# acerbilab/pyvbmc

Measured on AMD Instinct MI355X. Metric: ELBO+entropy evals/sec at D=10, K=50, N=400, Ns=1e6 (1e6-sample-equivalent evals/s), higher is better.
Workload: dtype f64; 1 GPU; BASELINE config 3 per GPU: D=10 K=50 N=400 S=1, Ns=1000000 MC samples per GPU (job Ns=1000000), value+grad _neg_elcbo with soft bounds, eps=philox; parallelism=single GPU

## Files before the change

### pyvbmc_amd/_lib.py

```python
import ctypes as C
import os
import sys
import threading
from pathlib import Path

import numpy as np

_HERE = Path(__file__).resolve().parent
LIB_PATH = Path(os.environ.get("VBMC_HIP_LIB", _HERE / "libvbmc_hip.so"))

EPS_RESIDENT, EPS_PHILOX = 0, 1
MEAN_ZERO, MEAN_CONST, MEAN_NEGQUAD = 0, 1, 2
E_ARG, E_HIP, E_RCCL, E_NODEV, E_UNSUP, E_NONFINITE = -1, -2, -3, -4, -5, -6
E_NOTPD = -8
W_GP_CHANGED = 1
W_NOT_FUSED = 2
T_ENTMC, T_GLJ, T_PDF, T_PREDICT, T_ELBO, T_PREDICT_VAR, T_GP_POST, T_IS_MCMC = range(8)


class VbmcHipError(RuntimeError):
    def __init__(self, code, msg):
        super().__init__(f"libvbmc_hip error {code}: {msg}")
        self.code = code

# ... 272 lines not shown
            if rc == E_ARG:
                raise ValueError(msg)
            if rc == E_NODEV:
                raise NoDeviceError(rc, msg)
            if rc == E_NOTPD:
                raise np.linalg.LinAlgError(msg)
            raise VbmcHipError(rc, msg)

    def device_info(self):
        name = C.create_string_buffer(256)
        cu, clk, mem = C.c_int(), C.c_int(), C.c_uint64()
        self.check(self._lib.vbmc_device_info(self._h, name, 256, C.byref(cu), C.byref(clk), C.byref(mem)))
        return {"name": name.value.decode(), "cu_count": cu.value, "clock_khz": clk.value,
                "hbm_bytes": mem.value}

    def host_affinity(self):
        b, n = C.c_int(), C.c_int()
        self.check(self._lib.vbmc_host_affinity(self._h, C.byref(b), C.byref(n)))
        return bool(b.value), n.value

    def synchronize(self):
        self.check(self._lib.vbmc_synchronize(self._h))

    def set_timing(self, on):
        self.check(self._lib.vbmc_set_timing(self._h, int(on) if on else 0))

    def set_option(self, key, value):
        self.check(self._lib.vbmc_set_option(self._h, key.encode(), int(value)))

    def last_entmc_plan(self):
        out = (C.c_int * 4)()
        self.check(self._lib.vbmc_last_entmc_plan(self._h, out))
        return {"kernel": ("valu", "ws", "small", "mfma", "adam_fused", "ws", "ws")[out[0]] if out[0] >= 0 else None, "rg": out[1],
                "chunks": out[2], "resident_draws": bool(out[3]), "span": out[0] in (5, 6), "adam_tail": out[0] == 6}

    def philox_normals(self, K, n_half, D, seed, row_begin=0, row_count=None):
        row_count = n_half - row_begin if row_count is None else row_count
        out = np.empty((K, row_count, D))
        self.check(self._lib.vbmc_philox_normals(self._h, K, n_half, D, C.c_uint64(seed), row_begin, row_count, ptr(out)))
        return out

    def armed_stats(self):
        out = (C.c_uint64 * 6)()
        self.check(self._lib.vbmc_armed_stats(self._h, out))
        return dict(zip(("hits", "cancels", "late", "ident_checked", "ident_bad", "lost"), (int(v) for v in out)))

    def last_elbo_raw(self, D, K):
        out = np.empty(1 + D * K + 2 * K + D)
        self.check(self._lib.vbmc_last_elbo_raw(self._h, ptr(out), out.size))
        return out

    def last_kernel_ms(self, which=T_ENTMC):
        v = C.c_double()
        self.check(self._lib.vbmc_last_kernel_ms(self._h, which, C.byref(v)))
        return v.value

    def last_host_us(self):
        out = np.zeros(5)
        self.check(self._lib.vbmc_last_host_us(self._h, ptr(out)))
        return out

    def last_step_marks(self):
        out = np.zeros(4)
        self.check(self._lib.vbmc_last_step_marks(self._h, ptr(out)))
        return {"gp_word_us": out[0], "entropy_word_us": out[1],
                "gp_sums_in": ("prep launch", "finish launch", "entropy launch")[int(out[2])]}

# ... 108 lines not shown
```

### pyvbmc_amd/csrc/common.h

```cpp
#pragma once
#include <hip/hip_runtime.h>
#include <chrono>

#include <cstdint>
#include <cstdio>
#include <string>
#include <vector>

#include "../../include/vbmc_hip.h"
#include "scratch.h"

struct ncclComm;

struct MixLayout {
  int D = 0, K = 0;
  int o_mup = 0;
  int o_mu = 0;
  int o_is2 = 0;
  int o_wc = 0;
  int o_rc = 0;
  int o_lrc = 0;
  int o_sig = 0;
  int o_w = 0;
  int o_lam = 0;
// ... 179 lines not shown
  size_t h_eps_cap = 0;
  size_t h_pinned_cap = 0;
  double* h_pack = nullptr;
  size_t h_pack_cap = 0;
  bool pack_in_flight = false;
  bool pack_valid = false;
  bool defer_mix_upload = false;
  double* hp_dev = nullptr;
  int timing = 0;
  double host_us[5] = {0, 0, 0, 0, 0};
  double step_marks[4] = {0, 0, 0, 0};
  int gp_where = 0;
  int opt_entmc_valu = 0;
  int opt_gp_ship = 1;
  int opt_entmc_mfma = 1;
  int opt_elbo_pregen = 1;
  int opt_elbo_ahead = 1;
  int opt_predict_dma = 1;
  int opt_predict_fused = 1;
  int opt_arm_late_test = 0;
  int opt_acq_poll = 1;
  int opt_is_mcmc_threads = 512;
  void (*release_cb)(void*) = nullptr;
  void* release_cb_user = nullptr;
  int opt_adam_fused = 1;
  int opt_adam_tail = 1;
  int opt_ident_test = 0;
  bool ident_retry = false;
  int opt_elbo_arm = 1;
  bool counted = false;
  int opt_ws_span = 1;
  int opt_ws_front = 0;
  int opt_ws_pad = -1;
  int opt_mix_bar = 1;
  double* h_pack_dev = nullptr;
  double* h_pack_dev_of = nullptr;
  std::vector<double> exp_eta;
  double exp_eta_sum = 0.0;
  bool exp_eta_valid = false;
  int last_plan[4] = {-1, 0, 0, 0};
  size_t last_raw_off = 0;
  int last_raw_n = 0;

  GpState gp;
  GpState gp_next;
  double* d_post_ws = nullptr;
  size_t d_post_ws_cap = 0;

  ncclComm* comm = nullptr;
  int rank = 0, world = 1;

  std::vector<const double*> gp_watch_ptrs;
  std::vector<int64_t> gp_watch_lens;
  uint64_t gp_watch_ck = 0;

  ElboScratch elbo;
  void* adam = nullptr;
  void* acq_is = nullptr;
  bool host_bound = false;
  int host_cpus = 0;
  void* randn_dev = nullptr;
  int randn_last_reused = 0;
  int opt_randn_dev = 1;
  void* xf = nullptr;
};
inline int ctx_cus(const vbmc_ctx* ctx) { return ctx->prop.multiProcessorCount > 0 ? ctx->prop.multiProcessorCount : 256; }
// ... 292 lines not shown
```

### pyvbmc_amd/csrc/ctx.hip

```cpp
#include <algorithm>
#include <cmath>
#include <cstdarg>
#include <cstdlib>
#include <cstring>

#include <sched.h>

#include <cctype>
#include <cstdio>

#include "common.h"

thread_local std::string g_create_err;

int vbmc_fail(vbmc_ctx* ctx, int code, const char* fmt, ...) {
  char buf[1024];
  va_list ap;
  va_start(ap, fmt);
  vsnprintf(buf, sizeof buf, fmt, ap);
  va_end(ap);
  if (ctx)
    ctx->err = buf;
  else
    g_create_err = buf;
// ... 57 lines not shown
  HIP_TRY(ctx, stream_wait(ctx));
  for (int i = 0; dst && i < k; ++i)
    if (dst[i]) memcpy(dst[i] + o, ctx->h_pinned + i * stride, sizeof(double) * count);
  return 0;
}

#include <atomic>
static std::atomic<int> g_live_ctx[64];
int vbmc_live_contexts_on(int device) { return device >= 0 && device < 64 ? g_live_ctx[device].load() : 2; }

static void options_from_env(vbmc_ctx* c) {
  const char* e = getenv("VBMC_ENTMC_KERNEL");
  c->opt_entmc_valu = (e && e[0] == 'v') ? 1 : 0;
  e = getenv("VBMC_ELBO_PREGEN");
  c->opt_elbo_pregen = !(e && e[0] == '0');
  e = getenv("VBMC_ELBO_AHEAD");
  c->opt_elbo_ahead = !(e && e[0] == '0');
  e = getenv("VBMC_ELBO_ARM");
  c->opt_elbo_arm = e ? atoi(e) : 1;
  e = getenv("VBMC_ACQ_POLL");
  c->opt_acq_poll = !(e && e[0] == '0');
  e = getenv("VBMC_ADAM_FUSED");
  c->opt_adam_fused = e ? atoi(e) : 1;
  e = getenv("VBMC_RANDN_DEVICE");
  c->opt_randn_dev = e ? (e[0] == '0' ? 0 : e[0] == '2' ? 2 : 1) : 1;
  e = getenv("VBMC_ADAM_TAIL");
  c->opt_adam_tail = e ? atoi(e) : 1;
  e = getenv("VBMC_WS_SPAN");
  c->opt_ws_span = !(e && e[0] == '0');
  e = getenv("VBMC_WS_FRONT");
  if (e) c->opt_ws_front = atoi(e);
  e = getenv("VBMC_WS_PAD");
  if (e) c->opt_ws_pad = atoi(e);
  e = getenv("VBMC_MIX_BAR");
  c->opt_mix_bar = !(e && e[0] == '0');
  e = getenv("VBMC_PREDICT_DMA");
  c->opt_predict_dma = !(e && e[0] == '0');
  e = getenv("VBMC_PREDICT_FUSED_FINISH");
  if (e) c->opt_predict_fused = atoi(e);
  e = getenv("VBMC_GP_SHIP");
  c->opt_gp_ship = !(e && e[0] == '0');
}

extern "C" {

int vbmc_abi_version(void) { return 2; }

int vbmc_device_count(int* n_out) {
  int n = 0;
  hipError_t e = hipGetDeviceCount(&n);
  if (e != hipSuccess) {
    n = 0;
    (void)hipGetLastError();
  }
  if (n_out) *n_out = n;
  return VBMC_OK;
}

}

static void bind_host_thread(vbmc_ctx* ctx) {
  const char* e = getenv("VBMC_HOST_AFFINITY");
  if (e && e[0] == '0') return;
  char bus[64] = {0};
  if (hipDeviceGetPCIBusId(bus, (int)sizeof(bus) - 1, ctx->device) != hipSuccess) {
    (void)hipGetLastError();
// ... 152 lines not shown
  if (clock_khz) *clock_khz = ctx->prop.clockRate;
  if (hbm_bytes) *hbm_bytes = (uint64_t)ctx->prop.totalGlobalMem;
  return VBMC_OK;
}

int vbmc_synchronize(vbmc_ctx* ctx) {
  if (!ctx) return VBMC_E_ARG;
  if (ctx->device < 0) return VBMC_OK;
  HIP_TRY(ctx, hipSetDevice(ctx->device));
  HIP_TRY(ctx, stream_wait(ctx));
  return VBMC_OK;
}

int vbmc_set_option(vbmc_ctx* ctx, const char* key, int value) {
  if (!ctx || !key) return VBMC_E_ARG;
  if (!strcmp(key, "arm_late_test")) {
    ctx->opt_arm_late_test = value;
    return VBMC_OK;
  }
  if (!strcmp(key, "ident_test")) {
    ctx->opt_ident_test = value;
    return VBMC_OK;
  }
  spec_disarm(ctx);
  if (!strcmp(key, "entmc_kernel")) ctx->opt_entmc_valu = value == 1;
  else if (!strcmp(key, "entmc_mfma")) ctx->opt_entmc_mfma = value != 0;
  else if (!strcmp(key, "gp_ship")) ctx->opt_gp_ship = value != 0;
  else if (!strcmp(key, "elbo_pregen")) ctx->opt_elbo_pregen = value != 0;
  else if (!strcmp(key, "elbo_ahead")) ctx->opt_elbo_ahead = value != 0;
  else if (!strcmp(key, "predict_dma")) ctx->opt_predict_dma = value != 0;
  else if (!strcmp(key, "predict_fused")) ctx->opt_predict_fused = value < 0 ? 0 : value > 2 ? 2 : value;
  else if (!strcmp(key, "mix_bar")) ctx->opt_mix_bar = value != 0;
  else if (!strcmp(key, "ws_span")) ctx->opt_ws_span = value != 0;
  else if (!strcmp(key, "ws_pad")) ctx->opt_ws_pad = value > 8 ? 8 : value;
  else if (!strcmp(key, "ws_front")) ctx->opt_ws_front = value < 0 ? 0 : value > 990 ? 990 : value;
  else if (!strcmp(key, "elbo_arm")) ctx->opt_elbo_arm = value < 0 ? 0 : value > 2 ? 2 : value;
  else if (!strcmp(key, "acq_poll")) ctx->opt_acq_poll = value != 0;
  else if (!strcmp(key, "is_mcmc_threads")) ctx->opt_is_mcmc_threads = value <= 256 ? 256 : value >= 768 ? 768 : 512;
  else if (!strcmp(key, "randn_device")) ctx->opt_randn_dev = value < 0 ? 0 : value > 3 ? 3 : value;
  else if (!strcmp(key, "adam_tail")) ctx->opt_adam_tail = value;
  else if (!strcmp(key, "adam_fused")) ctx->opt_adam_fused = value;
  else return vbmc_fail(ctx, VBMC_E_ARG, "vbmc_set_option: unknown key '%s'", key);
  return VBMC_OK;
}

int vbmc_set_gp_watch(vbmc_ctx* ctx, const double* const* ptrs, const int64_t* lens, int n, uint64_t expected) {
  if (!ctx || n < 0 || (n > 0 && (!ptrs || !lens))) return VBMC_E_ARG;
  ctx->gp_watch_ptrs.assign(ptrs, ptrs + n);
  ctx->gp_watch_lens.assign(lens, lens + n);
  ctx->gp_watch_ck = expected;
  return VBMC_OK;
}

int vbmc_host_checksum(const double* const* ptrs, const int64_t* lens, int n, uint64_t* out) {
  if (!ptrs || !lens || n < 0 || !out) return VBMC_E_ARG;
  uint64_t s = 0;
  for (int a = 0; a < n; ++a) {
    if (!ptrs[a] || lens[a] < 0) return VBMC_E_ARG;
    s += (pack_checksum(ptrs[a], (size_t)lens[a]) + (uint64_t)lens[a]) * (0xD1B54A32D192ED03ull + 2ull * (uint64_t)a);
  }
  *out = s;
  return VBMC_OK;
}

int vbmc_last_entmc_plan(const vbmc_ctx* ctx, int out[4]) {
  if (!ctx || !out) return VBMC_E_ARG;
// ... 413 lines not shown
```

### pyvbmc_amd/csrc/entropy.hip

```cpp
#include <cstdlib>

#include <algorithm>

#include "common.h"
#include "fastmath.h"
#include "entropy_args.h"
#include "philox.h"
#ifdef FIN_TIMES
__device__ unsigned long long g_glj_stamp;
#define GLJ_STAMP() (g_glj_stamp = wall_clock64())
#endif
#include "glj_block.h"

namespace {

constexpr int WG = 256;
constexpr int WAVES = WG / 64;

__device__ inline double wave_sum(double v) {
  return fm::wave_sum_dpp(v);
}


template <int DP>
// ... 350 lines not shown
  a.row_count = row_count;
  a.seed = seed;
  a.eps_mode = eps_mode;
  a.want_grad = want_grad;
  const bool ws = use_ws_kernel(ctx, D, K);
  const int cus = ctx_cus(ctx);
  p.inv_ns = 1.0 / (double)ns_per_comp;
  int rows_per_wg = WG;
  a.rg = 1;
  size_t n_table = 0;
  if (ws) {
    const int64_t total_rows = row_count * K;
    int64_t rg = (total_rows + 64 * 2 * cus - 1) / (64 * 2 * cus);
    if (rg < 1) rg = 1;
    if (rg > 16) rg = 16;
    a.rg = (int)rg;
    rows_per_wg = 64 * a.rg;
    n_table = (size_t)K * (size_t)ws_table_rows(K) * (size_t)(p.DP + 6);
  }
  a.chunks = (int)((row_count + rows_per_wg - 1) / rows_per_wg);
  if (a.chunks < 1) a.chunks = 1;
  if (ws) {
    const int64_t slots = (int64_t)cus * ws_min_waves(p.DP, ws_ktmax_for(K), want_grad != 0);
    const int64_t fit = slots / K;
    if (fit >= 1 && a.chunks > fit && (int64_t)K * (a.chunks - 1) <= slots) {
      const int64_t rg2 = (row_count + 64 * fit - 1) / (64 * fit);
      if (rg2 <= 24) {
        a.rg = (int)rg2;
        rows_per_wg = 64 * a.rg;
        a.chunks = (int)((row_count + rows_per_wg - 1) / rows_per_wg);
      }
    }
  }
  a.pair_cus = 0;
  if (ws) {
    const int64_t total = (int64_t)K * a.chunks;
    if (ws_min_waves(p.DP, ws_ktmax_for(K), want_grad != 0) == 2 && total > cus && total <= 2 * (int64_t)cus)
      a.pair_cus = cus;
  }
  EntArgs at_launch = a;
  {
    const size_t n_eps = (size_t)K * (size_t)row_count * D;
    if (eps_mode == VBMC_EPS_PHILOX && ctx->opt_elbo_pregen && n_eps > 0 && n_eps <= ((size_t)1 << 28)) {
      at_launch.eps_mode = VBMC_EPS_RESIDENT;
      at_launch.eps = (const double*)ctx;
    }
    if (at_launch.eps_mode == VBMC_EPS_RESIDENT && at_launch.eps == nullptr) at_launch.eps = (const double*)ctx;
  }
  p.kernel = !ws                                                          ? EntKernel::Valu
             : entmc_small_applies(at_launch, p.DP)                       ? EntKernel::Small
             : ctx->opt_entmc_mfma && entmc_mfma_applies(at_launch, p.DP) ? EntKernel::Mfma
                                                                          : EntKernel::Ws;
  a.sp = WsSpan();
  a.gp_wgs = 0;
  p.gp_in_ws = false;
  if (p.kernel == EntKernel::Ws && ctx->opt_ws_span) {
    const int waves = ws_min_waves(p.DP, ws_ktmax_for(K), want_grad != 0);
    WsSpan sp;
    sp.cus = cus;
    sp.nb = (int)((row_count + 63) >> 6);
    sp.pad = ctx->opt_ws_pad >= 0 ? ctx->opt_ws_pad : 3;
    sp.T = (int64_t)K * sp.nbv();
    sp.front = ctx->opt_ws_front > 0 ? ctx->opt_ws_front : ws_front_default(p.DP, ws_ktmax_for(K));
    static const int slots_env = [] {
      const char* e = getenv("VBMC_WS_GP_SLOTS");
      return e ? atoi(e) : 0;
// ... 132 lines not shown
  return 0;
}

GenSlice entmc_ahead_slice(vbmc_ctx* ctx, const EntPlan& p) {
  const double frac_end = 1.0;
  const EntArgs& a = p.a;
  GenSlice none;
  if (!ctx->opt_elbo_ahead || a.eps == nullptr || a.eps != ctx->d_epsgen[ctx->gen_cur]) return none;
  const int D = ctx->D, K = ctx->K, other = 1 - ctx->gen_cur;
  const size_t n_eps = (size_t)K * (size_t)a.row_count * D;
  if (ctx->d_epsgen_cap[other] < n_eps || !ctx->d_epsgen[other]) {
    if (ctx->d_epsgen[other]) return none;
    if (ensure_dev(ctx, &ctx->d_epsgen[other], &ctx->d_epsgen_cap[other], n_eps)) return none;
  }
  vbmc_ctx::AheadDraws& ah = ctx->ahead;
  ah.seed = a.seed + 1;
  ah.K = K;
  ah.D = D;
  ah.rows = a.row_count;
  ah.n_half = a.n_half;
  ah.row_begin = a.row_begin;
  ah.buf = other;
  ah.frac = frac_end;
  ah.valid = true;
  return make_gen_slice(ctx->d_epsgen[other], K, D, a.row_count, a.n_half, a.row_begin, ah.seed, nullptr, 0.0, frac_end);
}

int entmc_launch_main(vbmc_ctx* ctx, const EntPlan& p) {
  const EntArgs& a = p.a;
  hipEvent_t e0 = ctx->timing ? ctx->ev[2 * T_ENTMC] : nullptr, e1 = ctx->timing ? ctx->ev[2 * T_ENTMC + 1] : nullptr;
  ctx->last_plan[0] = (int)p.kernel;
  ctx->last_plan[1] = a.rg;
  ctx->last_plan[2] = a.chunks;
  ctx->last_plan[3] = a.eps_mode == VBMC_EPS_RESIDENT ? 1 : 0;
  const bool bracket = ctx->timing && (p.kernel == EntKernel::Valu || p.kernel == EntKernel::Small);
  if (bracket) HIP_TRY(ctx, hipEventRecord(ctx->ev[2 * T_ENTMC], ctx->stream));
  switch (p.kernel) {
    case EntKernel::Small: launch_entmc_small(ctx->stream, a, p.DP, p.table); break;
    case EntKernel::Mfma: launch_entmc_mfma(ctx->stream, a, p.DP, p.table, e0, e1); break;
    case EntKernel::Ws:
    case EntKernel::WsSpan:
      switch (p.DP) {
#define VBMC_CASE_WS(dp) case dp: launch_entmc_ws_dp##dp(ctx->stream, a, p.table, e0, e1); break;
        VBMC_WS_DPS(VBMC_CASE_WS)
#undef VBMC_CASE_WS
      }
      break;
    case EntKernel::Valu:
      switch (p.DP) {
#define VBMC_CASE_VALU(dp) case dp: launch_entmc_dp<dp>(ctx, a); break;
        VBMC_WS_DPS(VBMC_CASE_VALU)
#undef VBMC_CASE_VALU
      }
      break;
    default: return vbmc_fail(ctx, VBMC_E_ARG, "entmc: plan names no entropy kernel (%d)", (int)p.kernel);
  }
  if (ctx->timing) {
    if (bracket) HIP_TRY(ctx, hipEventRecord(ctx->ev[2 * T_ENTMC + 1], ctx->stream));
    ctx->ev_valid[T_ENTMC] = true;
  }
  HIP_TRY(ctx, hipGetLastError());
  return 0;
}

namespace {
__global__ __launch_bounds__(256) void eps_gen_kernel(GenSlice g) { gen_slice_block(g, blockIdx.x, threadIdx.x); }
}
// ... 104 lines not shown
```

### pyvbmc_amd/csrc/entropy_args.h

```cpp
#pragma once
#include "common.h"

struct WsSpan {
  int cus = 0;
  int pb = 0;
  int front = 0;
  int nb = 0;
  int pad = 0;
  int R = 0;
  int64_t T = 0;
  __host__ __device__ int nbv() const { return nb + pad; }
  __host__ __device__ int n_parts() const { return cus + pb; }
  __host__ __device__ int64_t W() const { return (int64_t)pb * 1000 + (int64_t)(cus - pb) * front; }
  __host__ __device__ int64_t cw(int u) const {
    return u < 2 * pb ? (int64_t)(u >> 1) * 1000 + (int64_t)(u & 1) * front : (int64_t)pb * 1000 + (int64_t)(u - 2 * pb) * front;
  }
  __host__ __device__ int64_t lo(int u) const { return cw(u) * T / W(); }
  __host__ __device__ int part_of(int64_t g) const {
    const int64_t c = ((g + 1) * W() - 1) / T;
    int u;
    if (c < (int64_t)pb * 1000) {
      const int p = (int)(c / 1000);
      u = 2 * p + ((c - (int64_t)p * 1000) >= front ? 1 : 0);
    } else {
      u = 2 * pb + (int)((c - (int64_t)pb * 1000) / front);
    }
    return u < n_parts() ? u : n_parts() - 1;
  }
  __host__ __device__ int part_of_block(int b) const { return b < cus ? (b < pb ? 2 * b : 2 * pb + (b - pb)) : 2 * (b - cus) + 1; }
};

struct EntArgs {
  const double* mix;
  MixLayout ml;
  const double* eps;
  int64_t eps_rows;
  int64_t n_half;
  int64_t row_begin;
  int64_t row_count;
  uint64_t seed;
  int eps_mode;
  int want_grad;
  double* partial;
  int chunks;
  int stride;
  int rg;
  const void* extra = nullptr;
  int extra_lds = 0;
  int gp_items = 0;
  PrepArgs gp;
  int pair_cus = 0;
  WsSpan sp;
  int gp_wgs = 0;
  const uint64_t* cancel = nullptr;
  const double* ship_src = nullptr;
  double* ship_dst = nullptr;
  int ship_n = 0;
  uint64_t* ship_flag = nullptr;
  uint64_t ship_seq = 0;
};

constexpr int ws_ktmax_for(int K) {
  const int KT = (K + 3) / 4;
  return KT <= 4 ? 4 : KT <= 8 ? 8 : KT <= 10 ? 10 : KT <= 13 ? 13 : KT <= 16 ? 16 : KT <= 20 ? 20 : KT <= 25 ? 25 : 32;
}
constexpr int ws_table_rows(int K) { return 4 * ws_ktmax_for(K); }
constexpr int ws_min_waves(int dp, int ktmax, bool grad) {
#ifdef VBMC_WS_FORCE_WAVES
  return VBMC_WS_FORCE_WAVES;
#else
  return (grad && 4 * dp + 3 * ktmax > 95) ? 1 : 2;
#endif
}

enum class EntKernel : int { Valu = 0, Ws = 1, Small = 2, Mfma = 3, AdamFused = 4, WsSpan = 5, AdamTail = 6 };

struct EntPlan {
  EntArgs a;
  EntKernel kernel = EntKernel::Valu;
  bool gp_in_ws = false;
  bool pregen_hit = false;
  int DP = 0;
  double inv_ns = 0.0;
  double* table = nullptr;
  bool tabled() const { return kernel != EntKernel::Valu; }
};

#define VBMC_WS_DPS(X) X(2) X(4) X(6) X(8) X(10) X(12) X(16) X(20) X(24) X(32)
inline int padded_d(int D) {
#define VBMC_PAD_D(dp) if (D <= dp) return dp;
  VBMC_WS_DPS(VBMC_PAD_D)
#undef VBMC_PAD_D
  return -1;
}
#define VBMC_DECL_WS(dp) \
  void launch_entmc_ws_dp##dp(hipStream_t st, const EntArgs& a, const double* d_table, hipEvent_t e0, hipEvent_t e1);
VBMC_WS_DPS(VBMC_DECL_WS)
#undef VBMC_DECL_WS

// ... 6 lines not shown
```

### pyvbmc_amd/csrc/entropy_ws.hip

```cpp
#include <hip/hip_ext.h>

#include "adam_dev.h"
#include "common.h"
#include "entropy_args.h"
#include "fastmath.h"
#include "glj_block.h"

#ifndef WS_EXP2_N
#define WS_EXP2_N VBMC_ENT_EXP2_N
#endif
constexpr int EN = WS_EXP2_N;
__device__ __forceinline__ double exp2_vc(double x, const double (&c)[EN]) {
  const double t = __builtin_rint(x);
  const double f = x - t;
  const int n = (int)t;
  double p = c[EN - 1];
#pragma unroll
  for (int i = EN - 2; i >= 0; --i) p = fma(p, f, c[i]);
  p = fma(p, f, 1.0);
  return __builtin_amdgcn_ldexp(p, n);
}
__device__ __forceinline__ void exp2_vc2(double x1, double x2, const double (&c)[EN], double& r1,
                                         double& r2) {
  const double t1 = __builtin_rint(x1), t2 = __builtin_rint(x2);
  const double f1 = x1 - t1, f2 = x2 - t2;
  const int n1 = (int)t1, n2 = (int)t2;
  double p1 = c[EN - 1], p2 = c[EN - 1];
#pragma unroll
  for (int i = EN - 2; i >= 0; --i) {
    p1 = fma(p1, f1, c[i]);
    p2 = fma(p2, f2, c[i]);
  }
  p1 = fma(p1, f1, 1.0);
// ... 5 lines not shown
__device__ const double kExp2C[EN] = VBMC_ENT_EXP2_COEFFS;
#elif WS_EXP2_N == 10
__device__ const double kExp2C[10] = {0x1.62e42fefa3a19p-1, 0x1.ebfbdff82c598p-3, 0x1.c6b08d703ce49p-5, 0x1.3b2ab6fba1ddap-7, 0x1.5d87fe9d7a584p-10, 0x1.430913096fd9fp-13, 0x1.ffcb54062e698p-17, 0x1.62bfd47773353p-20, 0x1.b675bca4eeebbp-24, 0x1.e6063f7217bc6p-28};
#elif WS_EXP2_N == 9
__device__ const double kExp2C[9] = {0x1.62e42fefa39f7p-1, 0x1.ebfbdff8149f2p-3, 0x1.c6b08d7044119p-5, 0x1.3b2ab72b175eep-7, 0x1.5d87fe908f88ap-10, 0x1.43088e257f341p-13, 0x1.ffcb76789860fp-17, 0x1.63ef969a64d3cp-20, 0x1.b6571de2f2351p-24};
#endif

#include "philox.h"

#ifndef VBMC_DP
#error "compile with -DVBMC_DP=<padded D>"
#endif

namespace {

constexpr int WG = 256;
constexpr int WAVES = WG / 64;

__device__ __forceinline__ double wave_sum(double v) { return fm::wave_sum_dpp(v); }

constexpr int ws_dmin(int dp) { return dp <= 12 ? dp - 1 : dp == 16 ? 13 : dp == 20 ? 17 : dp == 24 ? 21 : 25; }

constexpr int ws_epi_cap_doubles(int dp, int ktmax, bool grad) { return (ws_min_waves(dp, ktmax, grad) >= 2 ? 44 : 100) * 1024 / 8; }
constexpr int ws_epi_nq(int dp, int ktmax, bool grad) {
  if (!grad) return 0;
  const int ni = 1 + 2 * dp + ktmax;
  for (int nq = 1; nq <= 3; ++nq)
    if (WAVES * ni * ((64 >> nq) + 1) <= ws_epi_cap_doubles(dp, ktmax, grad)) return nq;
  return 0;
}
constexpr int ws_epi_doubles(int dp, int ktmax, bool grad) {
  const int nq = ws_epi_nq(dp, ktmax, grad);
  return nq == 0 ? 0 : WAVES * (1 + 2 * dp + ktmax) * ((64 >> nq) + 1);
}

#if defined(WS_TIMES) && VBMC_DP == 10
__device__ unsigned long long g_ws_times[1024 * 4];
#define WS_STAMP(i) do { if (threadIdx.x == 0) g_ws_times[(blockIdx.y * gridDim.x + blockIdx.x) * 4 + (i)] = wall_clock64(); } while (0)
#else
#define WS_STAMP(i) (void)0
#endif
constexpr int ws_dprev(int dp) { return dp <= 12 ? dp - 2 : dp == 16 ? 12 : dp == 20 ? 16 : dp == 24 ? 20 : 24; }
template <int DP, int KTMAX, bool GRAD, bool PHILOX, int STAGE = 0>
__global__ __launch_bounds__(WG, ws_min_waves(DP, KTMAX, GRAD)) void entmc_ws_kernel(
    EntArgs a, const double* __restrict__ T) {
  constexpr int TS = DP + 6;
  __shared__ double sQ[2][WAVES][2][64];
  constexpr int GB = 4;
  __shared__ __attribute__((aligned(16))) double sE[PHILOX ? GB : 2][DP][64];
  __shared__ double sRed[WAVES][2 * DP + 1];
  extern __shared__ double dyn[];
  constexpr int EPI = ws_epi_doubles(DP, KTMAX, GRAD);
  double* sW = dyn + EPI;

  constexpr bool EXTRA_ROW = GRAD && !PHILOX;
  const bool span = a.sp.cus > 0;
  if constexpr (EXTRA_ROW) {
    if (a.extra != nullptr && (span ? (int)blockIdx.x == a.sp.n_parts() + (a.gp_items > 0 ? a.gp_wgs : 0) : blockIdx.y == 0)) {
      if (span || blockIdx.x == 0) {
        const adam_dev::AdamDev& pa = *(const adam_dev::AdamDev*)a.extra;
        if (a.gp_items > 0 && a.gp.done.dev) {
          if (threadIdx.x == 0) {
            const unsigned long long t0 = wall_clock64();
            while (__hip_atomic_load(a.gp.done.flag, __ATOMIC_RELAXED, __HIP_MEMORY_SCOPE_AGENT) != a.gp.done.seq) {
              if (wall_clock64() - t0 > 2000000ull) {
                atomicOr(pa.status, 8);
                break;
              }
              __builtin_amdgcn_s_sleep(8);
            }
            __builtin_amdgcn_fence(__ATOMIC_ACQUIRE, "agent");
          }
          __syncthreads();
        }
        if (a.extra_lds > 0) adam_dev::adam_pre_body<true>(pa, dyn, &sRed[0][0], pa.pre);
        else adam_dev::adam_pre_body<false>(pa, nullptr, &sRed[0][0], pa.pre);
      }
      return;
    }
  }
  if (a.cancel != nullptr && __hip_atomic_load(a.cancel, __ATOMIC_RELAXED, __HIP_MEMORY_SCOPE_SYSTEM) == ~(uint64_t)0) return;
  if (a.gp_items > 0 && (span ? (int)blockIdx.x >= a.sp.n_parts() && (int)blockIdx.x < a.sp.n_parts() + a.gp_wgs : blockIdx.y == gridDim.y - 1)) {
    const int first = span ? (int)blockIdx.x - a.sp.n_parts() : (int)blockIdx.x, step = span ? a.gp_wgs : (int)gridDim.x;
    if (a.gp.x_lds) {
      if (first < a.gp_items) glj_stage_x(a.gp, dyn);
      for (int it = first; it < a.gp_items; it += step) {
        glj_block<true, DP, ws_dmin(DP), true>(a.gp, it, dyn);
        __syncthreads();
      }
    } else {
      for (int it = first; it < a.gp_items; it += step) {
        glj_block<false, DP, ws_dmin(DP), true>(a.gp, it, dyn);
        __syncthreads();
      }
    }
    return;
  }
  const int D = a.ml.D;
  constexpr int KT = KTMAX, K4 = KT * 4;
  int64_t g_lo, g_hi;
  int nb, part = 0, chunk_slot = 0, j_chunk = 0;
  int nbv;
  if (span) {
    nb = a.sp.nb;
    nbv = a.sp.nbv();
    part = a.sp.part_of_block((int)blockIdx.x);
    g_lo = a.sp.lo(part);
    g_hi = a.sp.lo(part + 1);
  } else {
    int j = (EXTRA_ROW && a.extra != nullptr) ? blockIdx.y - 1 : blockIdx.y, chunk = blockIdx.x;
    if (a.pair_cus > 0) {
      const int total = a.ml.K * a.chunks, b = j * a.chunks + chunk;
      const int paired = total - a.pair_cus;
      if (paired > 0 && b < 2 * a.pair_cus) {
        const int m = b < a.pair_cus ? b : b - a.pair_cus;
        const int item = m < paired ? 2 * m + (b >= a.pair_cus ? 1 : 0) : paired + m;
        j = item / a.chunks;
        chunk = item - j * a.chunks;
      }
    }
    nb = (int)((a.row_count + 63) >> 6);
    nbv = nb;
    chunk_slot = chunk;
    j_chunk = j;
    const int64_t i0 = (int64_t)chunk * a.rg;
    g_lo = (int64_t)j * nb + (i0 < nb ? i0 : nb);
    g_hi = (int64_t)j * nb + (i0 + a.rg < nb ? i0 + a.rg : nb);
  }
  const int tid = threadIdx.x, lane = tid & 63;
  const int wave = __builtin_amdgcn_readfirstlane(tid >> 6);
  WS_STAMP(0);
  constexpr bool eps_exact = !PHILOX && STAGE != 0;

  double ec[EN];
  {
    int vz;
    asm volatile("v_mov_b32 %0, 0" : "=v"(vz));
#pragma unroll
    for (int i = 0; i < EN; ++i) ec[i] = kExp2C[i + vz];
  }
  WS_STAMP(1);
  bool first_stretch = true;
  for (int64_t g = g_lo; g < g_hi || (first_stretch && !span);) {
  first_stretch = false;
  const int j = span ? (int)(g / nbv) : j_chunk;
  const int ib0 = (int)(g - (int64_t)j * nbv);
  if (span && ib0 >= nb) {
    g = (int64_t)(j + 1) * nbv;
    continue;
  }
  const int n_it = g < g_hi ? (int)((g_hi - g < nb - ib0) ? g_hi - g : nb - ib0) : 0;
  const int slot = span ? part - a.sp.part_of((int64_t)j * nbv) : chunk_slot;
  const double sig_j = a.mix[a.ml.o_sig + j];
  const double sj2 = sig_j * sig_j;
  const double two_sj = 2.0 * sig_j;
  const double* Tj = T + (size_t)j * K4 * TS;
  double slog_acc = 0.0;
  double mu_acc[DP], lam_acc[DP], Wacc[KTMAX];
#pragma unroll
  for (int d = 0; d < DP; ++d) mu_acc[d] = lam_acc[d] = 0.0;
#pragma unroll
  for (int kk = 0; kk < KTMAX; ++kk) Wacc[kk] = 0.0;

// ... 74 lines not shown
        for (int d = 0; d < DP; ++d)
          if (d < D) e[d] = rp[d];
      }
    } else {
      constexpr int NP = DP / 2;
      const int nbk = (D + 3) / 4;
      if ((it % GB) == 0) {
        const int nb = min(GB, n_it - it);
        __syncthreads();
        for (int q = wave; q < nb * nbk; q += WAVES) {
          const int bq = q / nbk, blk = q - bq * nbk;
          const int64_t il = ((int64_t)(ib0 + it + bq) << 6) + lane;
          const uint64_t grow = (uint64_t)j * (uint64_t)a.n_half + (uint64_t)(a.row_begin + il);
          double z[4];
          philox_normal_quad(grow, (uint32_t)blk, a.seed, z);
#pragma unroll
          for (int c = 0; c < 4; ++c)
            if (4 * blk + c < DP) sE[bq][4 * blk + c][lane] = z[c];
        }
        __syncthreads();
      }
      (void)NP;
#pragma unroll
      for (int d = 0; d < DP; ++d)
        if (valid && d < D) e[d] = sE[it % GB][d][lane];
    }
    double e2 = 0.0;
#pragma unroll
    for (int d = 0; d < DP; ++d) e2 = fma(e[d], e[d], e2);
    const double b = sj2 * e2;

    int zoff;
    asm volatile("s_mov_b32 %0, 0" : "=s"(zoff));
    const double* Tw = Tj + (size_t)wave * TS + zoff;

    double qp = 0.0, qm = 0.0;
    double rp_[KTMAX], rm_[KTMAX];
    constexpr int NR1 = DP + 3;
    double cur[NR1], nxt[NR1];
    {
      const double* tr = Tw;
#pragma unroll
      for (int i = 0; i < NR1; ++i) cur[i] = tr[i];
    }
#pragma unroll
    for (int kk = 0; kk < KTMAX; ++kk) {
      {
        __builtin_amdgcn_s_waitcnt(0xC07F);
        __builtin_amdgcn_sched_barrier(0);
        if (kk + 1 < KTMAX) {
          const double* tn = Tw + (size_t)(4 * (kk + 1)) * TS;
#pragma unroll
          for (int i = 0; i < NR1; ++i) nxt[i] = tn[i];
        }
        __builtin_amdgcn_sched_barrier(0);
        double c = 0.0;
#pragma unroll
        for (int d = 0; d < DP; ++d) c = fma(cur[d], e[d], c);
        const double sp = fma(two_sj, c, b);
        const double sm = fma(-two_sj, c, b);
        double rp, rm;
        exp2_vc2(fma(cur[DP + 1], sp, cur[DP + 0]), fma(cur[DP + 1], sm, cur[DP + 0]), ec, rp, rm);
        rp_[kk] = rp;
        rm_[kk] = rm;
        qp = fma(cur[DP + 2], rp, qp);
        qm = fma(cur[DP + 2], rm, qm);
#pragma unroll
        for (int i = 0; i < NR1; ++i) cur[i] = nxt[i];
      }
    }
    const int buf = it & 1;
    sQ[buf][wave][0][lane] = qp;
    sQ[buf][wave][1][lane] = qm;
    if constexpr (eps_exact) asm volatile("s_waitcnt vmcnt(0)" ::: "memory");
    __syncthreads();
    qp = (sQ[buf][0][0][lane] + sQ[buf][1][0][lane]) + (sQ[buf][2][0][lane] + sQ[buf][3][0][lane]);
    qm = (sQ[buf][0][1][lane] + sQ[buf][1][1][lane]) + (sQ[buf][2][1][lane] + sQ[buf][3][1][lane]);

    if (wave < 2) {
      const double qv = valid ? (wave == 0 ? qp : qm) : 1.0;
      lmant *= __builtin_amdgcn_frexp_mant(qv);
      lexp += __builtin_amdgcn_frexp_exp(qv);
      if ((it & (LOGB - 1)) == LOGB - 1 || it + 1 == n_it) {
        slog_acc += fma((double)lexp, 0x1.62e42fefa39efp-1, fm::log_fast(lmant));
        lmant = 1.0;
        lexp = 0;
      }
    }
    if (GRAD) {
      const double ip = valid ? fm::rcp_fast(qp) : 0.0;
      const double im = valid ? fm::rcp_fast(qm) : 0.0;
      double sgs = 0.0, sgd = 0.0;
      double Td[DP];
#pragma unroll
      for (int d = 0; d < DP; ++d) Td[d] = 0.0;
      constexpr int NR2 = DP + 4;
      double c2[NR2], n2[NR2];
      {
        const double* tr = Tw;
#pragma unroll
        for (int d = 0; d < DP; ++d) c2[d] = tr[d];
        c2[DP + 3] = tr[DP + 3];
      }
#pragma unroll
      for (int kk = 0; kk < KTMAX; ++kk) {
        {
          __builtin_amdgcn_s_waitcnt(0xC07F);
          __builtin_amdgcn_sched_barrier(0);
          if (kk + 1 < KTMAX) {
            const double* tn = Tw + (size_t)(4 * (kk + 1)) * TS;
#pragma unroll
            for (int d = 0; d < DP; ++d) n2[d] = tn[d];
            n2[DP + 3] = tn[DP + 3];
          }
          __builtin_amdgcn_sched_barrier(0);
          const double t2 = rm_[kk] * im;
          const double ts = fma(rp_[kk], ip, t2), td = fma(rp_[kk], ip, -t2);
          Wacc[kk] += ts;
          sgs = fma(ts, c2[DP + 3], sgs);
          const double gd = td * c2[DP + 3];
          sgd += gd;
#pragma unroll
          for (int d = 0; d < DP; ++d) Td[d] = fma(gd, c2[d], Td[d]);
#pragma unroll
          for (int d = 0; d < DP; ++d) c2[d] = n2[d];
          c2[DP + 3] = n2[DP + 3];
        }
      }
      const double cs = sig_j * sgs, cd = sig_j * sgd;
#pragma unroll
      for (int d = 0; d < DP; ++d) {
        mu_acc[d] = fma(e[d], cd, mu_acc[d]);
        lam_acc[d] = fma(e[d], fma(e[d], cs, Td[d]), lam_acc[d]);
      }
    }
  }

  WS_STAMP(2);
  if constexpr (EPI > 0) {
    constexpr int NQ = ws_epi_nq(DP, KTMAX, GRAD);
    constexpr int GL = 1 << NQ, NV = 64 / GL;
    constexpr int NI = 1 + 2 * DP + KTMAX, RS = NV + 1;
    static_assert(NQ >= 1 && NQ <= 3 && WAVES * NI * RS == EPI, "epilogue buffer");
    auto group = [](double v) {
      v += fm::dpp_get<0xB1, 0xf>(v);
      if constexpr (NQ >= 2) v += fm::dpp_get<0x4E, 0xf>(v);
      if constexpr (NQ >= 3) v += fm::dpp_get<0x141, 0xf>(v);
      return v;
    };
    {
      double* mine = dyn + (size_t)wave * NI * RS + (lane / GL);
      const bool wr = (lane & (GL - 1)) == 0;
      double v = group(slog_acc);
      if (wr) mine[0] = v;
#pragma unroll
      for (int d = 0; d < DP; ++d) {
        v = group(mu_acc[d]);
        if (wr) mine[(1 + d) * RS] = v;
        v = group(lam_acc[d]);
        if (wr) mine[(1 + DP + d) * RS] = v;
      }
#pragma unroll
      for (int kk = 0; kk < KTMAX; ++kk) {
        v = group(Wacc[kk]);
        if (wr) mine[(1 + 2 * DP + kk) * RS] = v;
      }
    }
    __syncthreads();
    for (int r = tid; r < WAVES * NI; r += WG) {
      const int wv = r / NI, it = r - wv * NI;
      const double* row = dyn + (size_t)r * RS;
      double x[NV];
#pragma unroll
      for (int l = 0; l < NV; ++l) x[l] = row[l];
      double s0 = 0.0, s1 = 0.0, s2 = 0.0, s3 = 0.0;
#pragma unroll
      for (int l = 0; l < NV; l += 4) {
        s0 += x[l];
        s1 += x[l + 1];
        s2 += x[l + 2];
        s3 += x[l + 3];
      }
      const double sum = (s0 + s1) + (s2 + s3);
      if (it <= 2 * DP) {
        sRed[wv][it] = sum;
      } else {
        const int kk = it - 1 - 2 * DP;
        sW[4 * kk + wv] = sum;
      }
    }
    __syncthreads();
  } else {
    {
      const double v = wave_sum(slog_acc);
      if (lane == 0) sRed[wave][0] = v;
    }
    if (GRAD) {
#pragma unroll
      for (int d = 0; d < DP; ++d) {
        const double vmu = wave_sum(mu_acc[d]);
        const double vlam = wave_sum(lam_acc[d]);
        if (lane == 0) {
          sRed[wave][1 + d] = vmu;
          sRed[wave][1 + DP + d] = vlam;
        }
      }
#pragma unroll
      for (int kk = 0; kk < KTMAX; ++kk)
        {
          const double v = wave_sum(Wacc[kk]);
          if (lane == 0) sW[4 * kk + wave] = v;
        }
    }
    __syncthreads();
  }

  WS_STAMP(3);
  double* out = a.partial + ((int64_t)j * a.chunks + slot) * a.stride;
  for (int t = tid; t < a.stride; t += WG) {
    double v = 0.0;
    if (t == 0) {
      for (int wv = 0; wv < WAVES; ++wv) v += sRed[wv][0];
    } else if (GRAD) {
      if (t <= D) {
        for (int wv = 0; wv < WAVES; ++wv) v += sRed[wv][t];
      } else if (t == D + 1) {
        for (int d = 0; d < D; ++d)
          for (int wv = 0; wv < WAVES; ++wv) v += sRed[wv][1 + DP + d];
      } else if (t < 2 * D + 2) {
        const int d = t - (D + 2);
        for (int wv = 0; wv < WAVES; ++wv) v += sRed[wv][1 + DP + d];
      } else {
        v = sW[t - (2 * D + 2)];
      }
    }
    out[t] = v;
  }
  if (span) {
    if (ib0 + n_it == nb)
      for (int t = tid; t < (a.chunks - 1 - slot) * a.stride; t += WG) out[a.stride + t] = 0.0;
    __syncthreads();
  }
  g += n_it;
  if (!span) break;
// ... 69 lines not shown
```

Measured before the change: 12140 evals/s.

## Assign wave roles by SIMD so component work balances across SIMDs

Each of the four waves in a workspace-entropy block now reads its hardware SIMD id and takes a role from it. Each role owns an uneven share of the mixture components, and the loop exits early once a role's share is done. The two lightest roles also take on the log-accumulation step, and filler blocks rotate roles so co-resident blocks on a CU spread the heavy work across SIMDs. This aims to balance VALU load per SIMD when K is not a multiple of four, at the cost of an extra shared-memory sync, a runtime trip bound inside the unrolled component loops, and register-pinning asm that may hurt scheduling.

```diff
diff --git a/pyvbmc_amd/_lib.py b/pyvbmc_amd/_lib.py
--- a/pyvbmc_amd/_lib.py
+++ b/pyvbmc_amd/_lib.py
@@ -328,7 +328,7 @@
         out = (C.c_int * 4)()
         self.check(self._lib.vbmc_last_entmc_plan(self._h, out))
         return {"kernel": ("valu", "ws", "small", "mfma", "adam_fused", "ws", "ws")[out[0]] if out[0] >= 0 else None, "rg": out[1],
-                "chunks": out[2], "resident_draws": bool(out[3]), "span": out[0] in (5, 6), "adam_tail": out[0] == 6}
+                "chunks": out[2], "resident_draws": bool(out[3] & 1), "roles": bool(out[3] & 2), "span": out[0] in (5, 6), "adam_tail": out[0] == 6}
 
     def philox_normals(self, K, n_half, D, seed, row_begin=0, row_count=None):
         row_count = n_half - row_begin if row_count is None else row_count
diff --git a/pyvbmc_amd/csrc/common.h b/pyvbmc_amd/csrc/common.h
--- a/pyvbmc_amd/csrc/common.h
+++ b/pyvbmc_amd/csrc/common.h
@@ -235,6 +235,7 @@
   int opt_ws_span = 1;
   int opt_ws_front = 0;
   int opt_ws_pad = -1;
+  int opt_ws_roles = 1;
   int opt_mix_bar = 1;
   double* h_pack_dev = nullptr;
   double* h_pack_dev_of = nullptr;
diff --git a/pyvbmc_amd/csrc/ctx.hip b/pyvbmc_amd/csrc/ctx.hip
--- a/pyvbmc_amd/csrc/ctx.hip
+++ b/pyvbmc_amd/csrc/ctx.hip
@@ -113,6 +113,8 @@
   if (e) c->opt_ws_front = atoi(e);
   e = getenv("VBMC_WS_PAD");
   if (e) c->opt_ws_pad = atoi(e);
+  e = getenv("VBMC_WS_ROLES");
+  c->opt_ws_roles = !(e && e[0] == '0');
   e = getenv("VBMC_MIX_BAR");
   c->opt_mix_bar = !(e && e[0] == '0');
   e = getenv("VBMC_PREDICT_DMA");
@@ -331,6 +333,7 @@
   else if (!strcmp(key, "predict_fused")) ctx->opt_predict_fused = value < 0 ? 0 : value > 2 ? 2 : value;
   else if (!strcmp(key, "mix_bar")) ctx->opt_mix_bar = value != 0;
   else if (!strcmp(key, "ws_span")) ctx->opt_ws_span = value != 0;
+  else if (!strcmp(key, "ws_roles")) ctx->opt_ws_roles = value != 0;
   else if (!strcmp(key, "ws_pad")) ctx->opt_ws_pad = value > 8 ? 8 : value;
   else if (!strcmp(key, "ws_front")) ctx->opt_ws_front = value < 0 ? 0 : value > 990 ? 990 : value;
   else if (!strcmp(key, "elbo_arm")) ctx->opt_elbo_arm = value < 0 ? 0 : value > 2 ? 2 : value;
diff --git a/pyvbmc_amd/csrc/entropy.hip b/pyvbmc_amd/csrc/entropy.hip
--- a/pyvbmc_amd/csrc/entropy.hip
+++ b/pyvbmc_amd/csrc/entropy.hip
@@ -406,6 +406,7 @@
       }
     }
   }
+  a.roles = ws && ctx->opt_ws_roles ? 1 : 0;
   a.pair_cus = 0;
   if (ws) {
     const int64_t total = (int64_t)K * a.chunks;
@@ -604,7 +605,7 @@
   ctx->last_plan[0] = (int)p.kernel;
   ctx->last_plan[1] = a.rg;
   ctx->last_plan[2] = a.chunks;
-  ctx->last_plan[3] = a.eps_mode == VBMC_EPS_RESIDENT ? 1 : 0;
+  ctx->last_plan[3] = (a.eps_mode == VBMC_EPS_RESIDENT ? 1 : 0) | ((p.kernel == EntKernel::Ws || p.kernel == EntKernel::WsSpan) && a.roles ? 2 : 0);
   const bool bracket = ctx->timing && (p.kernel == EntKernel::Valu || p.kernel == EntKernel::Small);
   if (bracket) HIP_TRY(ctx, hipEventRecord(ctx->ev[2 * T_ENTMC], ctx->stream));
   switch (p.kernel) {
diff --git a/pyvbmc_amd/csrc/entropy_args.h b/pyvbmc_amd/csrc/entropy_args.h
--- a/pyvbmc_amd/csrc/entropy_args.h
+++ b/pyvbmc_amd/csrc/entropy_args.h
@@ -52,6 +52,7 @@
   int pair_cus = 0;
   WsSpan sp;
   int gp_wgs = 0;
+  int roles = 0;
   const uint64_t* cancel = nullptr;
   const double* ship_src = nullptr;
   double* ship_dst = nullptr;
@@ -65,6 +66,19 @@
   return KT <= 4 ? 4 : KT <= 8 ? 8 : KT <= 10 ? 10 : KT <= 13 ? 13 : KT <= 16 ? 16 : KT <= 20 ? 20 : KT <= 25 ? 25 : 32;
 }
 constexpr int ws_table_rows(int K) { return 4 * ws_ktmax_for(K); }
+constexpr int ws_kt_role(int K, int r) { return K > r ? (K - r + 3) / 4 : 0; }
+constexpr int ws_ktmin_for(int ktmax) {
+  return ktmax <= 4 ? 1 : ktmax <= 8 ? 4 : ktmax <= 10 ? 8 : ktmax <= 13 ? 10 : ktmax <= 16 ? 13 : ktmax <= 20 ? 16 : ktmax <= 25 ? 20 : 25;
+}
+constexpr bool ws_kt_roles_cover(int kmax) {
+  for (int K = 1; K <= kmax; ++K) {
+    if (K >= 4 && ws_kt_role(K, 3) < ws_ktmin_for(ws_ktmax_for(K))) return false;
+    if (ws_kt_role(K, 0) + ws_kt_role(K, 1) + ws_kt_role(K, 2) + ws_kt_role(K, 3) != K) return false;
+    if (ws_kt_role(K, 0) > ws_ktmax_for(K) || ws_kt_role(K, 3) > ws_kt_role(K, 2) || ws_kt_role(K, 2) > ws_kt_role(K, 1)) return false;
+  }
+  return true;
+}
+static_assert(ws_kt_roles_cover(128), "the four roles own every component once, each at least ws_ktmin_for; roles 2 and 3 are the lightest");
 constexpr int ws_min_waves(int dp, int ktmax, bool grad) {
 #ifdef VBMC_WS_FORCE_WAVES
   return VBMC_WS_FORCE_WAVES;
diff --git a/pyvbmc_amd/csrc/entropy_ws.hip b/pyvbmc_amd/csrc/entropy_ws.hip
--- a/pyvbmc_amd/csrc/entropy_ws.hip
+++ b/pyvbmc_amd/csrc/entropy_ws.hip
@@ -1,4 +1,6 @@
 #include <hip/hip_ext.h>
+
+#include <type_traits>
 
 #include "adam_dev.h"
 #include "common.h"
@@ -70,6 +72,21 @@
 constexpr int ws_epi_doubles(int dp, int ktmax, bool grad) {
   const int nq = ws_epi_nq(dp, ktmax, grad);
   return nq == 0 ? 0 : WAVES * (1 + 2 * dp + ktmax) * ((64 >> nq) + 1);
+}
+
+template <int KK, int KTMIN, int KTMAX, class F>
+__device__ __forceinline__ void ws_for_owned(int kt, F&& f) {
+  if constexpr (KK < KTMAX) {
+    if constexpr (KK >= KTMIN)
+      if (KK == kt) return;
+    f(std::integral_constant<int, KK>());
+    ws_for_owned<KK + 1, KTMIN, KTMAX>(kt, f);
+  }
+}
+template <int N>
+__device__ __forceinline__ void ws_keep(const double (&r)[N]) {
+#pragma unroll
+  for (int i = 0; i < N; ++i) asm volatile("" : : "s"(r[i]));
 }
 
 #if defined(WS_TIMES) && VBMC_DP == 10
@@ -87,6 +104,7 @@
   constexpr int GB = 4;
   __shared__ __attribute__((aligned(16))) double sE[PHILOX ? GB : 2][DP][64];
   __shared__ double sRed[WAVES][2 * DP + 1];
+  __shared__ int sSimd[WAVES];
   extern __shared__ double dyn[];
   constexpr int EPI = ws_epi_doubles(DP, KTMAX, GRAD);
   double* sW = dyn + EPI;
@@ -139,9 +157,11 @@
   int64_t g_lo, g_hi;
   int nb, part = 0, chunk_slot = 0, j_chunk = 0;
   int nbv;
+  bool filler = false;
   if (span) {
     nb = a.sp.nb;
     nbv = a.sp.nbv();
+    filler = (int)blockIdx.x >= a.sp.cus;
     part = a.sp.part_of_block((int)blockIdx.x);
     g_lo = a.sp.lo(part);
     g_hi = a.sp.lo(part + 1);
@@ -150,6 +170,7 @@
     if (a.pair_cus > 0) {
       const int total = a.ml.K * a.chunks, b = j * a.chunks + chunk;
       const int paired = total - a.pair_cus;
+      filler = b >= a.pair_cus;
       if (paired > 0 && b < 2 * a.pair_cus) {
         const int m = b < a.pair_cus ? b : b - a.pair_cus;
         const int item = m < paired ? 2 * m + (b >= a.pair_cus ? 1 : 0) : paired + m;
@@ -167,6 +188,17 @@
   }
   const int tid = threadIdx.x, lane = tid & 63;
   const int wave = __builtin_amdgcn_readfirstlane(tid >> 6);
+  int role = wave;
+  if (a.roles) {
+    const int simd = (int)__builtin_amdgcn_s_getreg(4 | (4 << 6) | (1 << 11));
+    if (lane == 0) sSimd[wave] = simd;
+    __syncthreads();
+    const int seen = (1 << sSimd[0]) | (1 << sSimd[1]) | (1 << sSimd[2]) | (1 << sSimd[3]);
+    role = __builtin_amdgcn_readfirstlane(seen == 0xF ? (simd + (filler ? 2 : 0)) & 3 : wave);
+  }
+  constexpr int KTMIN = ws_ktmin_for(KTMAX);
+  const int kt_own = ws_kt_role(a.ml.K, role);
+  const int kt_r = __builtin_amdgcn_readfirstlane(a.roles ? (kt_own > KTMIN ? kt_own : KTMIN) : KTMAX);
   WS_STAMP(0);
   constexpr bool eps_exact = !PHILOX && STAGE != 0;
 
@@ -307,19 +339,22 @@
 
     int zoff;
     asm volatile("s_mov_b32 %0, 0" : "=s"(zoff));
-    const double* Tw = Tj + (size_t)wave * TS + zoff;
+    const double* Tw = Tj + (size_t)role * TS + zoff;
 
     double qp = 0.0, qm = 0.0;
     double rp_[KTMAX], rm_[KTMAX];
     constexpr int NR1 = DP + 3;
-    double cur[NR1], nxt[NR1];
+    double cur[NR1];
     {
       const double* tr = Tw;
 #pragma unroll
       for (int i = 0; i < NR1; ++i) cur[i] = tr[i];
     }
-#pragma unroll
-    for (int kk = 0; kk < KTMAX; ++kk) {
+    int kt1;
+    asm volatile("s_mov_b32 %0, %1" : "=s"(kt1) : "s"(kt_r));
+    ws_for_owned<0, KTMIN, KTMAX>(kt1, [&](auto kc) __attribute__((always_inline)) {
+      constexpr int kk = decltype(kc)::value;
+      double nxt[NR1];
       {
         __builtin_amdgcn_s_waitcnt(0xC07F);
         __builtin_amdgcn_sched_barrier(0);
@@ -342,18 +377,19 @@
         qm = fma(cur[DP + 2], rm, qm);
 #pragma unroll
         for (int i = 0; i < NR1; ++i) cur[i] = nxt[i];
-      }
-    }
+        if (kk + 1 < KTMAX && kk + 1 >= KTMIN) ws_keep(cur);
+      }
+    });
     const int buf = it & 1;
-    sQ[buf][wave][0][lane] = qp;
-    sQ[buf][wave][1][lane] = qm;
+    sQ[buf][role][0][lane] = qp;
+    sQ[buf][role][1][lane] = qm;
     if constexpr (eps_exact) asm volatile("s_waitcnt vmcnt(0)" ::: "memory");
     __syncthreads();
     qp = (sQ[buf][0][0][lane] + sQ[buf][1][0][lane]) + (sQ[buf][2][0][lane] + sQ[buf][3][0][lane]);
     qm = (sQ[buf][0][1][lane] + sQ[buf][1][1][lane]) + (sQ[buf][2][1][lane] + sQ[buf][3][1][lane]);
 
-    if (wave < 2) {
-      const double qv = valid ? (wave == 0 ? qp : qm) : 1.0;
+    if (role >= 2) {
+      const double qv = valid ? (role == 2 ? qp : qm) : 1.0;
       lmant *= __builtin_amdgcn_frexp_mant(qv);
       lexp += __builtin_amdgcn_frexp_exp(qv);
       if ((it & (LOGB - 1)) == LOGB - 1 || it + 1 == n_it) {
@@ -370,15 +406,18 @@
 #pragma unroll
       for (int d = 0; d < DP; ++d) Td[d] = 0.0;
       constexpr int NR2 = DP + 4;
-      double c2[NR2], n2[NR2];
+      double c2[NR2];
       {
         const double* tr = Tw;
 #pragma unroll
         for (int d = 0; d < DP; ++d) c2[d] = tr[d];
         c2[DP + 3] = tr[DP + 3];
       }
-#pragma unroll
-      for (int kk = 0; kk < KTMAX; ++kk) {
+      int kt2;
+      asm volatile("s_mov_b32 %0, %1" : "=s"(kt2) : "s"(kt_r));
+      ws_for_owned<0, KTMIN, KTMAX>(kt2, [&](auto kc) __attribute__((always_inline)) {
+        constexpr int kk = decltype(kc)::value;
+        double n2[NR2];
         {
           __builtin_amdgcn_s_waitcnt(0xC07F);
           __builtin_amdgcn_sched_barrier(0);
@@ -400,8 +439,13 @@
 #pragma unroll
           for (int d = 0; d < DP; ++d) c2[d] = n2[d];
           c2[DP + 3] = n2[DP + 3];
-        }
-      }
+          if (kk + 1 < KTMAX && kk + 1 >= KTMIN) {
+#pragma unroll
+            for (int d = 0; d < DP; ++d) asm volatile("" : : "s"(c2[d]));
+            asm volatile("" : : "s"(c2[DP + 3]));
+          }
+        }
+      });
       const double cs = sig_j * sgs, cd = sig_j * sgd;
 #pragma unroll
       for (int d = 0; d < DP; ++d) {
@@ -424,7 +468,7 @@
       return v;
     };
     {
-      double* mine = dyn + (size_t)wave * NI * RS + (lane / GL);
+      double* mine = dyn + (size_t)role * NI * RS + (lane / GL);
       const bool wr = (lane & (GL - 1)) == 0;
       double v = group(slog_acc);
       if (wr) mine[0] = v;
@@ -468,7 +512,7 @@
   } else {
     {
       const double v = wave_sum(slog_acc);
-      if (lane == 0) sRed[wave][0] = v;
+      if (lane == 0) sRed[role][0] = v;
     }
     if (GRAD) {
 #pragma unroll
@@ -476,15 +520,15 @@
         const double vmu = wave_sum(mu_acc[d]);
         const double vlam = wave_sum(lam_acc[d]);
         if (lane == 0) {
-          sRed[wave][1 + d] = vmu;
-          sRed[wave][1 + DP + d] = vlam;
+          sRed[role][1 + d] = vmu;
+          sRed[role][1 + DP + d] = vlam;
         }
       }
 #pragma unroll
       for (int kk = 0; kk < KTMAX; ++kk)
         {
           const double v = wave_sum(Wacc[kk]);
-          if (lane == 0) sW[4 * kk + wave] = v;
+          if (lane == 0) sW[4 * kk + role] = v;
         }
     }
     __syncthreads();
```

Result: faster. 12270 evals/s, median of 6 (+1.1%).
